# OFA-Sys/ONE-PEACE

Measured on NVIDIA H100. Metric: encoder_samples_per_sec, higher is better.
Workload: dtype bf16

## Files before the change

### one_peace_b200/csrc/gemm_wgmma.cu

```cuda
#include "common.cuh"
#include "gemm.h"

#include <mutex>

namespace opb {

constexpr int kBlockM = 128;
constexpr int kBlockN = 256;
constexpr int kBlockK = 64;
constexpr int kStages = 4;
constexpr int kABytes = kBlockM * kBlockK * 2;
constexpr int kBBytes = kBlockN * kBlockK * 2;
constexpr int kStageBytes = kABytes + kBBytes;
constexpr int kThreads = 384;
constexpr int kBandM = 8;
constexpr int kResidBatch = 16;

struct EpiOperands {
  float2 row[kBlockM];
  float colsum[kBlockN], bias[kBlockN], gamma[kBlockN], colscale[kBlockN];
};
constexpr int kStagerThreads = 96;
constexpr int kSmemBytes = kStages * kStageBytes + 1024 + 2 * sizeof(EpiOperands) + 1024;

struct GemmGeom {
  int M, N, K;
  int kb_inner;
  int num_k_blocks;
  int groups;
  int a_group_c0;
  int b_group_rows;
  int a_mn;
  int b_mn;
  int kb_per_piece;
  int m_pad;
  float* split_ws;
};

OPB_DEVICE void fence_acc(float (&d)[128]) {
#pragma unroll
  for (int i = 0; i < 128; ++i) asm volatile("" : "+f"(d[i])::"memory");
}

template <int TA, int TB>
OPB_DEVICE void wgmma_m64n256k16(float (&d)[128], uint64_t desc_a, uint64_t desc_b, uint32_t scale_d) {
  asm volatile(
      "{\n\t"
      ".reg .pred p;\n\t"
      "setp.ne.b32 p, %130, 0;\n\t"
      "wgmma.mma_async.sync.aligned.m64n256k16.f32.bf16.bf16 "
      "{"
      "%0, %1, %2, %3, %4, %5, %6, %7, %8, %9, %10, %11, %12, %13, %14, %15, "
      "%16, %17, %18, %19, %20, %21, %22, %23, %24, %25, %26, %27, %28, %29, %30, %31, "
      "%32, %33, %34, %35, %36, %37, %38, %39, %40, %41, %42, %43, %44, %45, %46, %47, "
      "%48, %49, %50, %51, %52, %53, %54, %55, %56, %57, %58, %59, %60, %61, %62, %63, "
      "%64, %65, %66, %67, %68, %69, %70, %71, %72, %73, %74, %75, %76, %77, %78, %79, "
      "%80, %81, %82, %83, %84, %85, %86, %87, %88, %89, %90, %91, %92, %93, %94, %95, "
      "%96, %97, %98, %99, %100, %101, %102, %103, %104, %105, %106, %107, %108, %109, %110, %111, "
      "%112, %113, %114, %115, %116, %117, %118, %119, %120, %121, %122, %123, %124, %125, %126, %127"
      "}, %128, %129, p, 1, 1, %131, %132;\n\t"
      "}\n"
      : "+f"(d[0]), "+f"(d[1]), "+f"(d[2]), "+f"(d[3]), "+f"(d[4]), "+f"(d[5]), "+f"(d[6]), "+f"(d[7]),
        "+f"(d[8]), "+f"(d[9]), "+f"(d[10]), "+f"(d[11]), "+f"(d[12]), "+f"(d[13]), "+f"(d[14]), "+f"(d[15]),
        "+f"(d[16]), "+f"(d[17]), "+f"(d[18]), "+f"(d[19]), "+f"(d[20]), "+f"(d[21]), "+f"(d[22]), "+f"(d[23]),
        "+f"(d[24]), "+f"(d[25]), "+f"(d[26]), "+f"(d[27]), "+f"(d[28]), "+f"(d[29]), "+f"(d[30]), "+f"(d[31]),
        "+f"(d[32]), "+f"(d[33]), "+f"(d[34]), "+f"(d[35]), "+f"(d[36]), "+f"(d[37]), "+f"(d[38]), "+f"(d[39]),
        "+f"(d[40]), "+f"(d[41]), "+f"(d[42]), "+f"(d[43]), "+f"(d[44]), "+f"(d[45]), "+f"(d[46]), "+f"(d[47]),
        "+f"(d[48]), "+f"(d[49]), "+f"(d[50]), "+f"(d[51]), "+f"(d[52]), "+f"(d[53]), "+f"(d[54]), "+f"(d[55]),
        "+f"(d[56]), "+f"(d[57]), "+f"(d[58]), "+f"(d[59]), "+f"(d[60]), "+f"(d[61]), "+f"(d[62]), "+f"(d[63]),
        "+f"(d[64]), "+f"(d[65]), "+f"(d[66]), "+f"(d[67]), "+f"(d[68]), "+f"(d[69]), "+f"(d[70]), "+f"(d[71]),
        "+f"(d[72]), "+f"(d[73]), "+f"(d[74]), "+f"(d[75]), "+f"(d[76]), "+f"(d[77]), "+f"(d[78]), "+f"(d[79]),
        "+f"(d[80]), "+f"(d[81]), "+f"(d[82]), "+f"(d[83]), "+f"(d[84]), "+f"(d[85]), "+f"(d[86]), "+f"(d[87]),
        "+f"(d[88]), "+f"(d[89]), "+f"(d[90]), "+f"(d[91]), "+f"(d[92]), "+f"(d[93]), "+f"(d[94]), "+f"(d[95]),
        "+f"(d[96]), "+f"(d[97]), "+f"(d[98]), "+f"(d[99]), "+f"(d[100]), "+f"(d[101]), "+f"(d[102]), "+f"(d[103]),
        "+f"(d[104]), "+f"(d[105]), "+f"(d[106]), "+f"(d[107]), "+f"(d[108]), "+f"(d[109]), "+f"(d[110]), "+f"(d[111]),
        "+f"(d[112]), "+f"(d[113]), "+f"(d[114]), "+f"(d[115]), "+f"(d[116]), "+f"(d[117]), "+f"(d[118]), "+f"(d[119]),
        "+f"(d[120]), "+f"(d[121]), "+f"(d[122]), "+f"(d[123]), "+f"(d[124]), "+f"(d[125]), "+f"(d[126]), "+f"(d[127])
      : "l"(desc_a), "l"(desc_b), "r"(scale_d), "n"(TA), "n"(TB));
}

template <bool kFusedVar = false>
OPB_DEVICE void load_ln_stats(const GemmEpilogue& ep, int row, int M, float& mu, float& rs) {
  mu = 0.f; rs = 1.f;
  const int rc = row < M ? row : M - 1;
  if (ep.ln_partial != nullptr) {
    float s1 = 0.f, s2 = 0.f;
#pragma unroll 8
    for (int p = 0; p < ep.ln_parts; ++p) {
      const float2 v = *reinterpret_cast<const float2*>(ep.ln_partial + (static_cast<long>(p) * M + rc) * 2);
      s1 += v.x; s2 += v.y;
    }
    mu = s1 / ep.ln_dim;
    const float ex2 = s2 / ep.ln_dim;
    const float var = kFusedVar ? fmaf(-mu, mu, ex2) : __fsub_rn(ex2, __fmul_rn(mu, mu));
    rs = rsqrtf(fmaxf(var, 0.f) + ep.ln_eps);
  } else if (ep.ln_mu != nullptr) {
    mu = ep.ln_mu[rc];
    rs = ep.ln_rstd[rc];
  }
}

OPB_DEVICE float2 ldf2(const float* p) { return *reinterpret_cast<const float2*>(p); }
OPB_DEVICE float quad_sum(float v) {
  v += __shfl_xor_sync(0xffffffffu, v, 1);
  return v + __shfl_xor_sync(0xffffffffu, v, 2);
}

template <int TA, int TB>
OPB_DEVICE void mainloop(float (&d)[128], uint8_t* smem, uint64_t* full, uint64_t* empty, int num_k_blocks, int cw,
                         uint32_t it0) {
  constexpr uint32_t step_a = TA ? 2048 : 32, step_b = TB ? 2048 : 32;
  const bool signal = (threadIdx.x & 31) == 0;
  for (int kb = 0; kb < num_k_blocks; ++kb) {
    const uint32_t it = it0 + kb;
    const uint32_t s = it % kStages;
    mbar_wait_quiet(&full[s], (it / kStages) & 1);
    const uint32_t sa = smem_u32(smem + s * kStageBytes) + cw * 8192;
    const uint32_t sb = smem_u32(smem + s * kStageBytes + kABytes);
    fence_acc(d);
    wgmma_fence();
#pragma unroll
    for (int k = 0; k < kBlockK / 16; ++k)
      wgmma_m64n256k16<TA, TB>(d, wgmma_desc_sw128(sa + k * step_a, 8192), wgmma_desc_sw128(sb + k * step_b, 8192),
                               (kb > 0 || k > 0) ? 1u : 0u);
    wgmma_commit();
    fence_acc(d);
    if (kb > 0) {
      wgmma_wait<1>();
      fence_acc(d);
      __syncwarp();
      if (signal) mbar_arrive(&empty[(it - 1) % kStages]);
    }
  }
  wgmma_wait<0>();
  fence_acc(d);
  __syncwarp();
  if (signal) mbar_arrive(&empty[(it0 + num_k_blocks - 1) % kStages]);
}

constexpr bool epi_staged(int epi) { return epi != EPI_LSE_PARTIAL && epi != EPI_SOFTMAX_GRAD; }

template <int EPI>
OPB_DEVICE void stage_epi_operands(EpiOperands* st, const GemmEpilogue& ep, const GemmGeom& geo, int m_blk, int n_blk, int grp,
                                   int t) {
  if (ep.ln_partial != nullptr || ep.ln_mu != nullptr) {
    for (int r = t; r < kBlockM; r += kStagerThreads) {
      float mu, rs;
      load_ln_stats<EPI == EPI_GEGLU_BF16 || EPI == EPI_RESID_F32>(ep, m_blk * kBlockM + r, geo.M, mu, rs);
      st->row[r] = make_float2(mu, rs);
    }
  }
  for (int c = t; c < kBlockN; c += kStagerThreads) {
    const int tc = n_blk * kBlockN + c;
    const bool ok = tc < geo.N;
    const int col = grp * geo.N + tc;
    st->colsum[c] = ok && ep.ln_colsum != nullptr ? ep.ln_colsum[col] : 0.f;
    st->bias[c] = ok && ep.bias != nullptr ? ep.bias[col] : 0.f;
    st->gamma[c] = ok && ep.gamma != nullptr ? ep.gamma[col] : 0.f;
    st->colscale[c] = ok && ep.colscale != nullptr ? ep.colscale[col] : 0.f;
  }
}

template <int EPI>
OPB_DEVICE void epilogue(const float (&d)[128], const GemmEpilogue& ep, const GemmGeom& geo, const EpiOperands* st, int m_blk,
                         int n_blk, int grp, int cw) {
  const int M = geo.M, N = geo.N;
  const int t = threadIdx.x & 127;
  const int lane = t & 31;
  const int quad = lane & 3;
  const int rloc = cw * 64 + (t >> 5) * 16 + (lane >> 2);
  const int rbase = m_blk * kBlockM + rloc;
  const int col0 = n_blk * kBlockN;
  const int gcol0 = grp * N;
#pragma unroll
  for (int h = 0; h < 2; ++h) {
    const int row = rbase + 8 * h;
    bool row_ok = row < M;
    if (ep.out_group > 0 && ep.out_group_valid > 0 && (row % ep.out_group) >= ep.out_group_valid) row_ok = false;
    long out_row = row;
    if (ep.out_group > 0) out_row = static_cast<long>(row / ep.out_group) * ep.out_group_stride + (row % ep.out_group) + ep.out_row_offset;
    long res_row = out_row;
    if (ep.resid_period > 0) res_row = (row % ep.resid_period) + ep.resid_row_offset;

    if constexpr (EPI == EPI_LSE_PARTIAL) {
      const float scale = *ep.scale_ptr;
      const int tgt = row + ep.target_offset;
      const int nv = ep.n_valid > 0 ? ep.n_valid : N;
      float m = -INFINITY;
#pragma unroll
      for (int j = 0; j < 32; ++j) {
        const int col = col0 + 8 * j + 2 * quad;
        if (col < nv) m = fmaxf(m, scale * d[4 * j + 2 * h]);
        if (col + 1 < nv) m = fmaxf(m, scale * d[4 * j + 2 * h + 1]);
      }
      float ssum = 0.f, zsum = 0.f, best = -INFINITY, ztgt = 0.f;
      int best_idx = 0, has_tgt = 0;
#pragma unroll
      for (int j = 0; j < 32; ++j) {
#pragma unroll
        for (int e = 0; e < 2; ++e) {
          const int col = col0 + 8 * j + 2 * quad + e;
          if (col < nv) {
            const float z = scale * d[4 * j + 2 * h + e];
            ssum += __expf(z - m);
            zsum += z;
            if (z > best) { best = z; best_idx = col; }
            if (col == tgt) { ztgt = z; has_tgt = 1; }
          }
        }
      }
#pragma unroll
      for (int o = 1; o <= 2; o <<= 1) {
        const float m2 = __shfl_xor_sync(0xffffffffu, m, o), s2 = __shfl_xor_sync(0xffffffffu, ssum, o);
        const float zs2 = __shfl_xor_sync(0xffffffffu, zsum, o), b2 = __shfl_xor_sync(0xffffffffu, best, o);
        const int i2 = __shfl_xor_sync(0xffffffffu, best_idx, o), h2 = __shfl_xor_sync(0xffffffffu, has_tgt, o);
        const float zt2 = __shfl_xor_sync(0xffffffffu, ztgt, o);
        const float mn = fmaxf(m, m2);
        ssum = (m > -INFINITY ? ssum * __expf(m - mn) : 0.f) + (m2 > -INFINITY ? s2 * __expf(m2 - mn) : 0.f);
        m = mn;
        zsum += zs2;
        if (b2 > best || (b2 == best && i2 < best_idx)) { best = b2; best_idx = i2; }
        if (h2) { ztgt = zt2; has_tgt = 1; }
      }
      if (row_ok && quad == 0) {
        float* w = ep.ws + (static_cast<long>(n_blk) * M + row) * 8;
        *reinterpret_cast<float4*>(w) = make_float4(m, ssum, zsum, best);
        *reinterpret_cast<float4*>(w + 4) = make_float4(__int_as_float(best_idx), ztgt, has_tgt ? 1.f : 0.f, 0.f);
      }
    } else if constexpr (EPI == EPI_SOFTMAX_GRAD) {
      const float scale = *ep.scale_ptr;
      const float gscale = scale * ep.coef;
      const int tgt = row + ep.target_offset;
      const float lse = row_ok ? ep.row_lse[row] : 0.f;
      const float hit = 1.f - ep.eps - ep.eps_i;
      const int nv = ep.n_valid > 0 ? ep.n_valid : N;
      float gz = 0.f;
#pragma unroll
      for (int j = 0; j < 32; ++j) {
        const int col = col0 + 8 * j + 2 * quad;
        if (!row_ok || col >= N) continue;
        float gq[2];
#pragma unroll
        for (int e = 0; e < 2; ++e) {
          const float z = scale * d[4 * j + 2 * h + e];
          float g = __expf(z - lse) - ep.eps_i;
          if (col + e == tgt) g -= hit;
          if (col + e >= nv) g = 0.f;
          gz += g * z;
          gq[e] = g * gscale;
        }
        *reinterpret_cast<uint32_t*>(reinterpret_cast<__nv_bfloat16*>(ep.out) + out_row * ep.ldo + col) = pack_bf16x2(gq[0], gq[1]);
      }
      gz = quad_sum(gz);
      if (row_ok && quad == 0) ep.ws[static_cast<long>(n_blk) * M + row] = gz;
    } else {
      const float2 mr = (ep.ln_partial != nullptr || ep.ln_mu != nullptr) ? st->row[rloc + 8 * h] : make_float2(0.f, 1.f);
      const float mu = mr.x, rs = mr.y;
      const bool has_ln = ep.ln_colsum != nullptr;
      float st_sum = 0.f, st_sq = 0.f;
      if constexpr (EPI == EPI_GEGLU_BF16) {
        __nv_bfloat16* out = reinterpret_cast<__nv_bfloat16*>(ep.out) + out_row * ep.ldo + n_blk * (kBlockN / 2);
#pragma unroll
        for (int j = 0; j < 16; ++j) {
          const int tc = 8 * j + 2 * quad;
          float g0 = d[4 * j + 2 * h], g1 = d[4 * j + 2 * h + 1];
          float l0 = d[4 * (j + 16) + 2 * h], l1 = d[4 * (j + 16) + 2 * h + 1];
          if (has_ln) {
            const float2 cg = ldf2(st->colsum + tc), cl = ldf2(st->colsum + tc + kBlockN / 2);
            g0 = rs * (g0 - mu * cg.x); g1 = rs * (g1 - mu * cg.y);
            l0 = rs * (l0 - mu * cl.x); l1 = rs * (l1 - mu * cl.y);
          }
          if (ep.bias != nullptr) {
            const float2 bg = ldf2(st->bias + tc), bl = ldf2(st->bias + tc + kBlockN / 2);
            g0 += bg.x; g1 += bg.y; l0 += bl.x; l1 += bl.y;
          }
          const float u0 = gelu_erf(g0) * l0, u1 = gelu_erf(g1) * l1;
          st_sum += u0 + u1;
          st_sq += u0 * u0 + u1 * u1;
          if (row_ok) *reinterpret_cast<uint32_t*>(out + tc) = pack_bf16x2(u0, u1);
        }
        st_sum = quad_sum(st_sum);
        st_sq = quad_sum(st_sq);
        if (row_ok && quad == 0 && ep.stats_out != nullptr) {
          *reinterpret_cast<float2*>(ep.stats_out + (static_cast<long>(n_blk * 2) * M + row) * 2) = make_float2(st_sum, st_sq);
          *reinterpret_cast<float2*>(ep.stats_out + (static_cast<long>(n_blk * 2 + 1) * M + row) * 2) = make_float2(0.f, 0.f);
        }
      } else {
#pragma unroll
        for (int jb = 0; jb < 32; jb += kResidBatch) {
          float2 res[kResidBatch];
          if constexpr (EPI == EPI_RESID_F32) {
            if (ep.resid != nullptr && row_ok) {
              const float* rp = ep.resid + res_row * ep.ldr + gcol0;
#pragma unroll
              for (int jj = 0; jj < kResidBatch; ++jj) {
                const int tc = col0 + 8 * (jb + jj) + 2 * quad;
                if (tc < N) res[jj] = ldf2(rp + tc);
              }
            }
          }
#pragma unroll
          for (int jj = 0; jj < kResidBatch; ++jj) {
            const int j = jb + jj;
            const int lc = 8 * j + 2 * quad;
            const int tc = col0 + lc;
            if (tc >= N) continue;
            const int col = gcol0 + tc;
            float x0 = d[4 * j + 2 * h], x1 = d[4 * j + 2 * h + 1];
            if (has_ln) {
              const float2 c = ldf2(st->colsum + lc);
              x0 = rs * (x0 - mu * c.x); x1 = rs * (x1 - mu * c.y);
            }
            if (ep.bias != nullptr) {
              const float2 b = ldf2(st->bias + lc);
              x0 += b.x; x1 += b.y;
            }
            if constexpr (EPI == EPI_STORE_BF16 || EPI == EPI_GELU_BF16) {
              if (ep.colscale != nullptr) {
                const float2 s = ldf2(st->colscale + lc);
                x0 *= s.x; x1 *= s.y;
              }
              if constexpr (EPI == EPI_GELU_BF16) { x0 = gelu_erf(x0); x1 = gelu_erf(x1); }
              if (row_ok) *reinterpret_cast<uint32_t*>(reinterpret_cast<__nv_bfloat16*>(ep.out) + out_row * ep.ldo + col) = pack_bf16x2(x0, x1);
            } else {
              if constexpr (EPI == EPI_RESID_F32) {
                if (ep.gamma != nullptr) {
                  const float2 g = ldf2(st->gamma + lc);
                  x0 *= g.x; x1 *= g.y;
                }
                if (ep.resid != nullptr && row_ok) {
                  x0 += res[jj].x; x1 += res[jj].y;
                }
                st_sum += x0 + x1;
                st_sq += x0 * x0 + x1 * x1;
                if (row_ok && ep.out_bf16 != nullptr)
                  *reinterpret_cast<uint32_t*>(reinterpret_cast<__nv_bfloat16*>(ep.out_bf16) + out_row * ep.ldo_bf16 + col) = pack_bf16x2(x0, x1);
              }
              if (row_ok) *reinterpret_cast<float2*>(reinterpret_cast<float*>(ep.out) + out_row * ep.ldo + col) = make_float2(x0, x1);
            }
          }
        }
        if constexpr (EPI == EPI_RESID_F32) {
          st_sum = quad_sum(st_sum);
          st_sq = quad_sum(st_sq);
          if (row_ok && quad == 0 && ep.stats_out != nullptr)
            *reinterpret_cast<float2*>(ep.stats_out + (static_cast<long>(n_blk) * M + row) * 2) = make_float2(st_sum, st_sq);
        }
      }
    }
  }
}

struct TileCoord {
  int piece, grp, m_blk, n_blk;
};
OPB_DEVICE TileCoord tile_coord(int unit, int num_m_tiles, int num_n_tiles, int groups) {
  const int per_group = num_m_tiles * num_n_tiles;
  TileCoord c;
  c.piece = unit / (per_group * groups);
  const int tile = unit - c.piece * per_group * groups;
  c.grp = tile / per_group;
  const int tin = tile - c.grp * per_group;
  const int band = tin / (kBandM * num_n_tiles);
  const int m0 = band * kBandM;
  const int band_rows = min(kBandM, num_m_tiles - m0);
  const int r = tin - m0 * num_n_tiles;
  c.m_blk = m0 + r % band_rows;
  c.n_blk = r / band_rows;
  return c;
}

template <int EPI>
__global__ void __launch_bounds__(kThreads, 1)
gemm_bf16_kernel(const __grid_constant__ CUtensorMap tm_a, const __grid_constant__ CUtensorMap tm_b, const GemmEpilogue ep,
                 const GemmGeom geo) {
  extern __shared__ __align__(1024) uint8_t smem_raw[];
  uint8_t* smem = smem_raw;
  if ((smem_u32(smem) & 1023u) != 0) __trap();
  uint64_t* full = reinterpret_cast<uint64_t*>(smem + kStages * kStageBytes);
  uint64_t* empty = full + kStages;
  uint64_t* epi_full = empty + kStages;
  uint64_t* epi_empty = epi_full + 2;
  EpiOperands* epi_ops = reinterpret_cast<EpiOperands*>(smem + kStages * kStageBytes + 1024);

  const int wg = threadIdx.x >> 7;
  const int num_m_tiles = (geo.M + kBlockM - 1) / kBlockM;
  const int num_n_tiles = (geo.N + kBlockN - 1) / kBlockN;
  const int pieces = geo.kb_per_piece > 0 ? (geo.num_k_blocks + geo.kb_per_piece - 1) / geo.kb_per_piece : 1;
  const int units = num_m_tiles * num_n_tiles * geo.groups * pieces;
  const bool staged = epi_staged(EPI) && geo.kb_per_piece == 0;

  if (threadIdx.x == 0) {
    tma_prefetch_desc(&tm_a);
    tma_prefetch_desc(&tm_b);
    for (int i = 0; i < kStages; ++i) {
      mbar_init(&full[i], 1);
      mbar_init(&empty[i], 8);
    }
    for (int i = 0; i < 2; ++i) {
      mbar_init(&epi_full[i], kStagerThreads);
      mbar_init(&epi_empty[i], 8);
    }
    fence_barrier_init();
  }
  __syncthreads();

  if (wg == 0) {
    asm volatile("setmaxnreg.dec.sync.aligned.u32 40;");
    if (threadIdx.x == 0) {
      uint32_t it = 0;
      for (int unit = blockIdx.x; unit < units; unit += gridDim.x) {
        const TileCoord tc = tile_coord(unit, num_m_tiles, num_n_tiles, geo.groups);
        const int kb0 = geo.kb_per_piece > 0 ? tc.piece * geo.kb_per_piece : 0;
        const int kb1 = geo.kb_per_piece > 0 ? min(geo.num_k_blocks, kb0 + geo.kb_per_piece) : geo.num_k_blocks;
        const int a_row = tc.m_blk * kBlockM;
        const int b_row = tc.grp * geo.b_group_rows + tc.n_blk * kBlockN;
        const int a_c0 = tc.grp * geo.a_group_c0;
        int kin = kb0 % geo.kb_inner, tap = kb0 / geo.kb_inner;
        for (int kb = kb0; kb < kb1; ++kb, ++it) {
          const uint32_t s = it % kStages;
          mbar_wait_quiet(&empty[s], ((it / kStages) & 1) ^ 1);
          uint8_t* sa = smem + s * kStageBytes;
          uint8_t* sb = sa + kABytes;
          mbar_arrive_expect_tx(&full[s], kStageBytes);
          if (geo.a_mn) {
#pragma unroll
            for (int i = 0; i < kBlockM / 64; ++i) tma_load_2d(&tm_a, &full[s], sa + i * 8192, a_row + 64 * i, kb * kBlockK);
          } else {
            tma_load_3d(&tm_a, &full[s], sa, a_c0 + kin * kBlockK, tap, a_row);
          }
          if (geo.b_mn) {
#pragma unroll
            for (int i = 0; i < kBlockN / 64; ++i) tma_load_2d(&tm_b, &full[s], sb + i * 8192, b_row + 64 * i, kb * kBlockK);
          } else {
            tma_load_2d(&tm_b, &full[s], sb, kb * kBlockK, b_row);
          }
          if (++kin == geo.kb_inner) { kin = 0; ++tap; }
        }
      }
    } else if (threadIdx.x >= 32 && staged) {
      uint32_t j = 0;
      for (int unit = blockIdx.x; unit < units; unit += gridDim.x, ++j) {
        const TileCoord tc = tile_coord(unit, num_m_tiles, num_n_tiles, geo.groups);
        mbar_wait_quiet(&epi_empty[j & 1], ((j >> 1) & 1) ^ 1);
        stage_epi_operands<EPI>(&epi_ops[j & 1], ep, geo, tc.m_blk, tc.n_blk, tc.grp, threadIdx.x - 32);
        mbar_arrive(&epi_full[j & 1]);
      }
    }
  } else {
    asm volatile("setmaxnreg.inc.sync.aligned.u32 232;");
    const int cw = wg - 1;
    float d[128];
#pragma unroll
    for (int i = 0; i < 128; ++i) d[i] = 0.f;
    uint32_t it = 0, j = 0;
    for (int unit = blockIdx.x; unit < units; unit += gridDim.x, ++j) {
      const TileCoord tc = tile_coord(unit, num_m_tiles, num_n_tiles, geo.groups);
      const int kb0 = geo.kb_per_piece > 0 ? tc.piece * geo.kb_per_piece : 0;
      const int kb1 = geo.kb_per_piece > 0 ? min(geo.num_k_blocks, kb0 + geo.kb_per_piece) : geo.num_k_blocks;
      if (geo.a_mn) {
        if (geo.b_mn) mainloop<1, 1>(d, smem, full, empty, kb1 - kb0, cw, it);
        else mainloop<1, 0>(d, smem, full, empty, kb1 - kb0, cw, it);
      } else {
        if (geo.b_mn) mainloop<0, 1>(d, smem, full, empty, kb1 - kb0, cw, it);
        else mainloop<0, 0>(d, smem, full, empty, kb1 - kb0, cw, it);
      }
      it += kb1 - kb0;
      if (geo.kb_per_piece > 0) {
        const int t = threadIdx.x & 127, lane = t & 31;
        const int r0 = tc.m_blk * kBlockM + cw * 64 + (t >> 5) * 16 + (lane >> 2);
        float* w = geo.split_ws + static_cast<long>(tc.piece) * geo.m_pad * geo.N;
#pragma unroll
        for (int h = 0; h < 2; ++h) {
#pragma unroll
          for (int c = 0; c < 32; ++c) {
            const int col = tc.n_blk * kBlockN + 8 * c + 2 * (lane & 3);
            if (col < geo.N)
              *reinterpret_cast<float2*>(w + static_cast<long>(r0 + 8 * h) * geo.N + col) = make_float2(d[4 * c + 2 * h], d[4 * c + 2 * h + 1]);
          }
        }
      } else if (staged) {
        mbar_wait_quiet(&epi_full[j & 1], (j >> 1) & 1);
        epilogue<EPI>(d, ep, geo, &epi_ops[j & 1], tc.m_blk, tc.n_blk, tc.grp, cw);
        __syncwarp();
        if ((threadIdx.x & 31) == 0) mbar_arrive(&epi_empty[j & 1]);
      } else {
        epilogue<EPI>(d, ep, geo, nullptr, tc.m_blk, tc.n_blk, tc.grp, cw);
      }
    }
  }
}

__global__ void __launch_bounds__(256)
gemm_split_epilogue_kernel(const GemmEpilogue ep, const GemmGeom geo, int pieces, int epi) {
  __shared__ float red[2][8];
  const int M = geo.M, N = geo.N;
  const int row = blockIdx.x;
  float mu, rs;
  if (ep.ln_partial != nullptr) {
    float s1 = 0.f, s2 = 0.f;
    for (int p = threadIdx.x; p < ep.ln_parts; p += blockDim.x) {
      const float2 v = *reinterpret_cast<const float2*>(ep.ln_partial + (static_cast<long>(p) * M + row) * 2);
      s1 += v.x; s2 += v.y;
    }
    s1 = warp_sum(s1); s2 = warp_sum(s2);
    if ((threadIdx.x & 31) == 0) { red[0][threadIdx.x >> 5] = s1; red[1][threadIdx.x >> 5] = s2; }
    __syncthreads();
    s1 = s2 = 0.f;
    for (int i = 0; i < 8; ++i) { s1 += red[0][i]; s2 += red[1][i]; }
    mu = s1 / ep.ln_dim;
    rs = rsqrtf(fmaxf(s2 / ep.ln_dim - mu * mu, 0.f) + ep.ln_eps);
  } else {
    load_ln_stats(ep, row, M, mu, rs);
  }
  const int t = blockIdx.y;
  const int col = t * kBlockN + threadIdx.x;
  const long slab = static_cast<long>(geo.m_pad) * N;
  float x = 0.f;
  if (col < N) {
    const float* w = geo.split_ws + static_cast<long>(row) * N + col;
    for (int p = 0; p < pieces; ++p) x += w[p * slab];
    if (ep.ln_colsum) x = rs * (x - mu * ep.ln_colsum[col]);
    if (ep.bias) x += ep.bias[col];
    if (epi == EPI_STORE_BF16) {
      if (ep.colscale) x *= ep.colscale[col];
      reinterpret_cast<__nv_bfloat16*>(ep.out)[static_cast<long>(row) * ep.ldo + col] = __float2bfloat16(x);
    } else {
      if (ep.gamma) x *= ep.gamma[col];
      if (ep.resid) x += ep.resid[static_cast<long>(row) * ep.ldr + col];
      reinterpret_cast<float*>(ep.out)[static_cast<long>(row) * ep.ldo + col] = x;
      if (ep.out_bf16) reinterpret_cast<__nv_bfloat16*>(ep.out_bf16)[static_cast<long>(row) * ep.ldo_bf16 + col] = __float2bfloat16(x);
    }
  }
  if (ep.stats_out != nullptr) {
    const float s1 = warp_sum(x), s2 = warp_sum(x * x);
    __syncthreads();
    if ((threadIdx.x & 31) == 0) { red[0][threadIdx.x >> 5] = s1; red[1][threadIdx.x >> 5] = s2; }
    __syncthreads();
    if (threadIdx.x == 0) {
      float a = 0.f, b = 0.f;
      for (int i = 0; i < 8; ++i) { a += red[0][i]; b += red[1][i]; }
      *reinterpret_cast<float2*>(ep.stats_out + (static_cast<long>(t) * M + row) * 2) = make_float2(a, b);
    }
  }
}

typedef CUresult (*PFN_encodeTiled)(CUtensorMap*, CUtensorMapDataType, cuuint32_t, void*, const cuuint64_t*,
                                    const cuuint64_t*, const cuuint32_t*, const cuuint32_t*, CUtensorMapInterleave,
                                    CUtensorMapSwizzle, CUtensorMapL2promotion, CUtensorMapFloatOOBfill);

static PFN_encodeTiled get_encode_fn() {
  static PFN_encodeTiled fn = nullptr;
  static std::once_flag once;
  std::call_once(once, [] {
    void* p = nullptr;
    cudaDriverEntryPointQueryResult qres;
    if (cudaGetDriverEntryPoint("cuTensorMapEncodeTiled", &p, cudaEnableDefault, &qres) == cudaSuccess &&
        qres == cudaDriverEntryPointSuccess) {
      fn = reinterpret_cast<PFN_encodeTiled>(p);
    }
  });
  return fn;
}

int make_tmap_bf16_2d(CUtensorMap* out, const void* ptr, uint64_t rows, uint64_t cols, uint64_t ld,
                      uint32_t box_rows) {
  PFN_encodeTiled enc = get_encode_fn();
  if (enc == nullptr) return OPB_ERR_CUDA;
  if ((reinterpret_cast<uintptr_t>(ptr) & 15) != 0 || (ld * 2) % 16 != 0) return OPB_ERR_INVALID;
  cuuint64_t gdim[2] = {cols, rows};
  cuuint64_t gstride[1] = {ld * 2};
  cuuint32_t box[2] = {static_cast<cuuint32_t>(kBlockK), box_rows};
  cuuint32_t estr[2] = {1, 1};
  CUresult r = enc(out, CU_TENSOR_MAP_DATA_TYPE_BFLOAT16, 2, const_cast<void*>(ptr), gdim, gstride, box, estr,
                   CU_TENSOR_MAP_INTERLEAVE_NONE, CU_TENSOR_MAP_SWIZZLE_128B, CU_TENSOR_MAP_L2_PROMOTION_L2_256B,
                   CU_TENSOR_MAP_FLOAT_OOB_FILL_NONE);
  return r == CUDA_SUCCESS ? OPB_OK : OPB_ERR_CUDA;
}

int make_tmap_bf16_3d(CUtensorMap* out, const void* ptr, uint64_t k_inner, uint64_t taps, uint64_t tap_stride,
                      uint64_t rows, uint64_t row_stride, uint32_t box_rows) {
  PFN_encodeTiled enc = get_encode_fn();
  if (enc == nullptr) return OPB_ERR_CUDA;
  if ((reinterpret_cast<uintptr_t>(ptr) & 15) != 0 || (tap_stride * 2) % 16 != 0 || (row_stride * 2) % 16 != 0)
    return OPB_ERR_INVALID;
  cuuint64_t gdim[3] = {k_inner, taps, rows};
  cuuint64_t gstride[2] = {tap_stride * 2, row_stride * 2};
  cuuint32_t box[3] = {static_cast<cuuint32_t>(kBlockK), 1, box_rows};
  cuuint32_t estr[3] = {1, 1, 1};
  CUresult r = enc(out, CU_TENSOR_MAP_DATA_TYPE_BFLOAT16, 3, const_cast<void*>(ptr), gdim, gstride, box, estr,
                   CU_TENSOR_MAP_INTERLEAVE_NONE, CU_TENSOR_MAP_SWIZZLE_128B, CU_TENSOR_MAP_L2_PROMOTION_L2_256B,
                   CU_TENSOR_MAP_FLOAT_OOB_FILL_NONE);
  return r == CUDA_SUCCESS ? OPB_OK : OPB_ERR_CUDA;
}

int make_tmap_bf16_batched(CUtensorMap* out, const void* ptr, uint64_t cols, uint64_t rows, uint64_t ld, uint64_t batches,
                           uint64_t batch_stride, uint32_t box_rows) {
  PFN_encodeTiled enc = get_encode_fn();
  if (enc == nullptr) return OPB_ERR_CUDA;
  if ((reinterpret_cast<uintptr_t>(ptr) & 15) != 0 || (ld * 2) % 16 != 0 || (batch_stride * 2) % 16 != 0)
    return OPB_ERR_INVALID;
  cuuint64_t gdim[3] = {cols, rows, batches};
  cuuint64_t gstride[2] = {ld * 2, batch_stride * 2};
  cuuint32_t box[3] = {static_cast<cuuint32_t>(kBlockK), box_rows, 1};
  cuuint32_t estr[3] = {1, 1, 1};
  CUresult r = enc(out, CU_TENSOR_MAP_DATA_TYPE_BFLOAT16, 3, const_cast<void*>(ptr), gdim, gstride, box, estr,
                   CU_TENSOR_MAP_INTERLEAVE_NONE, CU_TENSOR_MAP_SWIZZLE_128B, CU_TENSOR_MAP_L2_PROMOTION_L2_256B,
                   CU_TENSOR_MAP_FLOAT_OOB_FILL_NONE);
  return r == CUDA_SUCCESS ? OPB_OK : OPB_ERR_CUDA;
}

template <int EPI>
static int launch_gemm(const CUtensorMap& ta, const CUtensorMap& tb, const GemmEpilogue& ep, const GemmGeom& geo,
                       cudaStream_t stream) {
  auto kern = gemm_bf16_kernel<EPI>;
  static int resident = 0;
  if (resident == 0) {
    if (cudaFuncSetAttribute(kern, cudaFuncAttributeMaxDynamicSharedMemorySize, kSmemBytes) != cudaSuccess)
      return OPB_ERR_CUDA;
    int per_sm = 0;
    if (cudaOccupancyMaxActiveBlocksPerMultiprocessor(&per_sm, kern, kThreads, kSmemBytes) != cudaSuccess || per_sm < 1)
      return OPB_ERR_CUDA;
    resident = per_sm * sm_count();
  }
  const int pieces = geo.kb_per_piece > 0 ? (geo.num_k_blocks + geo.kb_per_piece - 1) / geo.kb_per_piece : 1;
  const long units = static_cast<long>((geo.M + kBlockM - 1) / kBlockM) * ((geo.N + kBlockN - 1) / kBlockN) * geo.groups * pieces;
  const unsigned grid = static_cast<unsigned>(units < resident ? units : resident);
  kern<<<grid, kThreads, kSmemBytes, stream>>>(ta, tb, ep, geo);
  return cudaGetLastError() == cudaSuccess ? OPB_OK : OPB_ERR_CUDA;
}

static int dispatch_gemm(int epi, const CUtensorMap& ta, const CUtensorMap& tb, const GemmEpilogue& ep, const GemmGeom& geo,
                         cudaStream_t stream) {
  switch (epi) {
    case EPI_STORE_BF16: return launch_gemm<EPI_STORE_BF16>(ta, tb, ep, geo, stream);
    case EPI_GELU_BF16: return launch_gemm<EPI_GELU_BF16>(ta, tb, ep, geo, stream);
    case EPI_GEGLU_BF16: return launch_gemm<EPI_GEGLU_BF16>(ta, tb, ep, geo, stream);
    case EPI_RESID_F32: return launch_gemm<EPI_RESID_F32>(ta, tb, ep, geo, stream);
    case EPI_STORE_F32: return launch_gemm<EPI_STORE_F32>(ta, tb, ep, geo, stream);
    case EPI_LSE_PARTIAL: return launch_gemm<EPI_LSE_PARTIAL>(ta, tb, ep, geo, stream);
    case EPI_SOFTMAX_GRAD: return launch_gemm<EPI_SOFTMAX_GRAD>(ta, tb, ep, geo, stream);
    default: return OPB_ERR_INVALID;
  }
}

struct ByteSpan {
  const char* begin;
  const char* end;
};
static ByteSpan row_span(const void* p, long lo, long hi, long ld, long cols, int esz) {
  const char* c = static_cast<const char*>(p);
  return {c + lo * ld * esz, c + (hi * ld + cols) * esz};
}
static bool spans_meet(const ByteSpan& a, const ByteSpan& b) { return a.begin < b.end && b.begin < a.end; }

static bool resid_aliasing_ok(const GemmEpilogue& ep, int M, long cols) {
  if (ep.resid == nullptr) return true;
  auto out_row = [&](long m) {
    return ep.out_group > 0 ? (m / ep.out_group) * ep.out_group_stride + m % ep.out_group + ep.out_row_offset : m;
  };
  const long g = ep.out_group > 0 ? ep.out_group : M, last = M - 1, q = last / g;
  const long corners[5] = {0, (g < M ? g : M) - 1, q * g, last, q > 0 ? q * g - 1 : 0};
  long lo = out_row(0), hi = lo;
  for (long m : corners) {
    lo = out_row(m) < lo ? out_row(m) : lo;
    hi = out_row(m) > hi ? out_row(m) : hi;
  }
  long rlo = lo, rhi = hi;
  if (ep.resid_period > 0) {
    rlo = ep.resid_row_offset;
    rhi = rlo + (ep.resid_period < M ? ep.resid_period : M) - 1;
  }
  const ByteSpan res = row_span(ep.resid, rlo, rhi, ep.ldr, cols, 4);
  if (ep.out_bf16 != nullptr && spans_meet(res, row_span(ep.out_bf16, lo, hi, ep.ldo_bf16, cols, 2))) return false;
  if (!spans_meet(res, row_span(ep.out, lo, hi, ep.ldo, cols, 4))) return true;
  return ep.resid == ep.out && ep.ldr == ep.ldo && ep.resid_period == 0;
}

static GemmGeom plain_geom(int M, int N, int K) {
  GemmGeom geo;
  geo.M = M; geo.N = N; geo.K = K;
  geo.num_k_blocks = (K + kBlockK - 1) / kBlockK;
  geo.kb_inner = geo.num_k_blocks;
  geo.groups = 1;
  geo.a_group_c0 = 0;
  geo.b_group_rows = 0;
  geo.a_mn = geo.b_mn = 0;
  geo.kb_per_piece = 0;
  geo.m_pad = 0;
  geo.split_ws = nullptr;
  return geo;
}

int gemm_bf16(const void* A, int lda, const void* B, int ldb, int M, int N, int K, int epi, const GemmEpilogue& ep,
              int cta_group, cudaStream_t stream) {
  if (M <= 0 || N <= 0 || K <= 0) return OPB_ERR_INVALID;
  if (K % 8 != 0 || N % 8 != 0 || lda % 8 != 0 || ldb % 8 != 0) return OPB_ERR_INVALID;
  if (epi == EPI_GEGLU_BF16 && N % kBlockN != 0) return OPB_ERR_INVALID;
  if (cta_group < 0 || cta_group > 2) return OPB_ERR_INVALID;
  if (epi == EPI_RESID_F32 && !resid_aliasing_ok(ep, M, N)) return OPB_ERR_INVALID;
  GemmGeom geo = plain_geom(M, N, K);
  const int m_tiles = (M + kBlockM - 1) / kBlockM, n_tiles = (N + kBlockN - 1) / kBlockN;
  const bool split_ok = (epi == EPI_RESID_F32 || (epi == EPI_STORE_BF16 && ep.stats_out == nullptr)) && ep.workspace != nullptr &&
                        ep.out_group == 0 && ep.resid_period == 0 && M <= 2 * kBlockM && geo.num_k_blocks >= 8;
  int pieces = 1;
  if (split_ok) {
    const long slab_bytes = static_cast<long>(m_tiles) * kBlockM * N * 4;
    pieces = sm_count() / (m_tiles * n_tiles);
    if (pieces > geo.num_k_blocks / 2) pieces = geo.num_k_blocks / 2;
    if (pieces > ep.workspace_bytes / slab_bytes) pieces = static_cast<int>(ep.workspace_bytes / slab_bytes);
    if (pieces >= 2) {
      geo.kb_per_piece = (geo.num_k_blocks + pieces - 1) / pieces;
      pieces = (geo.num_k_blocks + geo.kb_per_piece - 1) / geo.kb_per_piece;
      geo.m_pad = m_tiles * kBlockM;
      geo.split_ws = reinterpret_cast<float*>(ep.workspace);
    }
  }
  CUtensorMap ta, tb;
  int rc = make_tmap_bf16_3d(&ta, A, K, 1, lda, M, lda, kBlockM);
  if (rc != OPB_OK) return rc;
  rc = make_tmap_bf16_2d(&tb, B, N, K, ldb, kBlockN);
  if (rc != OPB_OK) return rc;
  rc = dispatch_gemm(epi, ta, tb, ep, geo, stream);
  if (rc != OPB_OK || geo.kb_per_piece == 0) return rc;
  gemm_split_epilogue_kernel<<<dim3(M, n_tiles), 256, 0, stream>>>(ep, geo, pieces, epi);
  return cudaGetLastError() == cudaSuccess ? OPB_OK : OPB_ERR_CUDA;
}

int gemm_bf16_t(const void* A, int lda, int a_mn, const void* B, int ldb, int b_mn, int M, int N, int K, int epi,
                const GemmEpilogue& ep, int cta_group, cudaStream_t stream) {
  if (M <= 0 || N <= 0 || K <= 0 || lda % 8 != 0 || ldb % 8 != 0 || N % 8 != 0) return OPB_ERR_INVALID;
  if (epi != EPI_STORE_BF16 && epi != EPI_STORE_F32) return OPB_ERR_INVALID;
  if ((!a_mn && K % 8 != 0) || (!b_mn && K % 8 != 0) || (a_mn && M % 8 != 0)) return OPB_ERR_INVALID;
  if (cta_group < 0 || cta_group > 2) return OPB_ERR_INVALID;
  GemmGeom geo = plain_geom(M, N, K);
  geo.a_mn = a_mn ? 1 : 0;
  geo.b_mn = b_mn ? 1 : 0;
  CUtensorMap ta, tb;
  int rc = a_mn ? make_tmap_bf16_2d(&ta, A, K, M, lda, 64) : make_tmap_bf16_3d(&ta, A, K, 1, lda, M, lda, kBlockM);
  if (rc != OPB_OK) return rc;
  rc = b_mn ? make_tmap_bf16_2d(&tb, B, K, N, ldb, 64) : make_tmap_bf16_2d(&tb, B, N, K, ldb, kBlockN);
  if (rc != OPB_OK) return rc;
  return dispatch_gemm(epi, ta, tb, ep, geo, stream);
}

int gemm_bf16_grouped_window(const void* X, const void* W, int rows, int groups, int c_pad, int taps, int n_per_group,
                             int epi, const GemmEpilogue& ep, cudaStream_t stream) {
  if (rows <= 0 || groups <= 0 || taps <= 0 || n_per_group <= 0) return OPB_ERR_INVALID;
  if (c_pad % kBlockK != 0 || n_per_group % 8 != 0 || n_per_group > kBlockN) return OPB_ERR_INVALID;
  if (epi == EPI_GEGLU_BF16 || epi == EPI_LSE_PARTIAL || epi == EPI_SOFTMAX_GRAD) return OPB_ERR_INVALID;
  if (epi == EPI_RESID_F32 && !resid_aliasing_ok(ep, rows, static_cast<long>(groups) * n_per_group)) return OPB_ERR_INVALID;
  GemmGeom geo = plain_geom(rows, n_per_group, taps * c_pad);
  geo.kb_inner = c_pad / kBlockK;
  geo.num_k_blocks = taps * geo.kb_inner;
  geo.groups = groups;
  geo.a_group_c0 = c_pad;
  geo.b_group_rows = n_per_group;
  const long row_stride = static_cast<long>(groups) * c_pad;
  CUtensorMap ta, tb;
  int rc = make_tmap_bf16_3d(&ta, X, row_stride, taps, row_stride, rows, row_stride, kBlockM);
  if (rc != OPB_OK) return rc;
  rc = make_tmap_bf16_2d(&tb, W, static_cast<uint64_t>(groups) * n_per_group, geo.K, geo.K, kBlockN);
  if (rc != OPB_OK) return rc;
  return dispatch_gemm(epi, ta, tb, ep, geo, stream);
}

}
```

Before: 762.9.

## Stage bf16 GEMM epilogue outputs through shared memory and TMA bulk stores

Adds a TMA-store variant of the persistent wgmma GEMM for bf16 epilogues (store, GELU, GEGLU). Each consumer warpgroup packs its output with stmatrix into a swizzled shared-memory staging buffer and issues 2D TMA stores, in place of scattered 4-byte global writes. To make room in shared memory the stage ring drops from 4 to 3, which reduces how far loads can run ahead of the math. A warpgroup barrier and a bulk-read wait guard reuse of the staging buffer.

After: 790.7, median of 6. +3.6%, better.

```diff
diff --git a/one_peace_b200/csrc/gemm_wgmma.cu b/one_peace_b200/csrc/gemm_wgmma.cu
--- a/one_peace_b200/csrc/gemm_wgmma.cu
+++ b/one_peace_b200/csrc/gemm_wgmma.cu
@@ -9,6 +9,7 @@
 constexpr int kBlockN = 256;
 constexpr int kBlockK = 64;
 constexpr int kStages = 4;
+constexpr int kStagesTmaOut = 3;
 constexpr int kABytes = kBlockM * kBlockK * 2;
 constexpr int kBBytes = kBlockN * kBlockK * 2;
 constexpr int kStageBytes = kABytes + kBBytes;
@@ -21,7 +22,14 @@
   float colsum[kBlockN], bias[kBlockN], gamma[kBlockN], colscale[kBlockN];
 };
 constexpr int kStagerThreads = 96;
-constexpr int kSmemBytes = kStages * kStageBytes + 1024 + 2 * sizeof(EpiOperands) + 1024;
+constexpr int kOutBoxBytes = 64 * 128;
+constexpr int kOutStageBytes = 4 * kOutBoxBytes;
+constexpr int smem_bytes(int stages, bool tma_out) {
+  return stages * kStageBytes + (tma_out ? 2 * kOutStageBytes : 0) + 1024 + 2 * sizeof(EpiOperands) + 1024;
+}
+constexpr int kSmemBytes = smem_bytes(kStages, false);
+constexpr int kSmemBytesTmaOut = smem_bytes(kStagesTmaOut, true);
+static_assert(kSmemBytesTmaOut <= 227 * 1024, "output staging does not fit next to the stage ring");
 
 struct GemmGeom {
   int M, N, K;
@@ -106,15 +114,15 @@
   return v + __shfl_xor_sync(0xffffffffu, v, 2);
 }
 
-template <int TA, int TB>
+template <int TA, int TB, int S>
 OPB_DEVICE void mainloop(float (&d)[128], uint8_t* smem, uint64_t* full, uint64_t* empty, int num_k_blocks, int cw,
                          uint32_t it0) {
   constexpr uint32_t step_a = TA ? 2048 : 32, step_b = TB ? 2048 : 32;
   const bool signal = (threadIdx.x & 31) == 0;
   for (int kb = 0; kb < num_k_blocks; ++kb) {
     const uint32_t it = it0 + kb;
-    const uint32_t s = it % kStages;
-    mbar_wait_quiet(&full[s], (it / kStages) & 1);
+    const uint32_t s = it % S;
+    mbar_wait_quiet(&full[s], (it / S) & 1);
     const uint32_t sa = smem_u32(smem + s * kStageBytes) + cw * 8192;
     const uint32_t sb = smem_u32(smem + s * kStageBytes + kABytes);
     fence_acc(d);
@@ -129,13 +137,49 @@
       wgmma_wait<1>();
       fence_acc(d);
       __syncwarp();
-      if (signal) mbar_arrive(&empty[(it - 1) % kStages]);
+      if (signal) mbar_arrive(&empty[(it - 1) % S]);
     }
   }
   wgmma_wait<0>();
   fence_acc(d);
   __syncwarp();
-  if (signal) mbar_arrive(&empty[(it0 + num_k_blocks - 1) % kStages]);
+  if (signal) mbar_arrive(&empty[(it0 + num_k_blocks - 1) % S]);
+}
+
+template <int kGroups>
+OPB_DEVICE void stage_out_row(uint32_t stage, int h, const uint32_t (&v)[kGroups]) {
+  const int lane = threadIdx.x & 31;
+  const int row = ((threadIdx.x & 127) >> 5) * 16 + 8 * h + (lane & 7);
+#pragma unroll
+  for (int q = 0; q < kGroups / 4; ++q) {
+    const int cg = 4 * q + (lane >> 3);
+    const uint32_t addr = stage + (cg >> 3) * kOutBoxBytes + sw128_off(row, cg & 7);
+    asm volatile("stmatrix.sync.aligned.m8n8.x4.shared.b16 [%0], {%1, %2, %3, %4};" ::"r"(addr), "r"(v[4 * q]),
+                 "r"(v[4 * q + 1]), "r"(v[4 * q + 2]), "r"(v[4 * q + 3]));
+  }
+}
+
+OPB_DEVICE void warpgroup_bar_sync(int cw) {
+  if (cw == 0) asm volatile("bar.sync 1, 128;" ::: "memory");
+  else asm volatile("bar.sync 2, 128;" ::: "memory");
+}
+
+OPB_DEVICE void acquire_out_stage(int cw) {
+  if ((threadIdx.x & 127) == 0) bulk_wait_read<0>();
+  warpgroup_bar_sync(cw);
+}
+
+OPB_DEVICE void store_out_tile(const CUtensorMap& tm_out, uint8_t* stage, int row0, int col0, int rows, int cols, int boxes,
+                               int cw) {
+  fence_proxy_async();
+  warpgroup_bar_sync(cw);
+  if ((threadIdx.x & 127) == 0) {
+    if (row0 < rows) {
+      for (int b = 0; b < boxes; ++b)
+        if (col0 + 64 * b < cols) tma_store_2d(&tm_out, stage + b * kOutBoxBytes, col0 + 64 * b, row0);
+    }
+    bulk_commit();
+  }
 }
 
 constexpr bool epi_staged(int epi) { return epi != EPI_LSE_PARTIAL && epi != EPI_SOFTMAX_GRAD; }
@@ -161,9 +205,9 @@
   }
 }
 
-template <int EPI>
-OPB_DEVICE void epilogue(const float (&d)[128], const GemmEpilogue& ep, const GemmGeom& geo, const EpiOperands* st, int m_blk,
-                         int n_blk, int grp, int cw) {
+template <int EPI, bool kTmaOut>
+OPB_DEVICE void epilogue(const float (&d)[128], const GemmEpilogue& ep, const GemmGeom& geo, const EpiOperands* st,
+                         uint32_t out_stage, int m_blk, int n_blk, int grp, int cw) {
   const int M = geo.M, N = geo.N;
   const int t = threadIdx.x & 127;
   const int lane = t & 31;
@@ -260,6 +304,7 @@
       float st_sum = 0.f, st_sq = 0.f;
       if constexpr (EPI == EPI_GEGLU_BF16) {
         __nv_bfloat16* out = reinterpret_cast<__nv_bfloat16*>(ep.out) + out_row * ep.ldo + n_blk * (kBlockN / 2);
+        uint32_t packed[16];
 #pragma unroll
         for (int j = 0; j < 16; ++j) {
           const int tc = 8 * j + 2 * quad;
@@ -277,8 +322,10 @@
           const float u0 = gelu_erf(g0) * l0, u1 = gelu_erf(g1) * l1;
           st_sum += u0 + u1;
           st_sq += u0 * u0 + u1 * u1;
-          if (row_ok) *reinterpret_cast<uint32_t*>(out + tc) = pack_bf16x2(u0, u1);
+          if constexpr (kTmaOut) packed[j] = pack_bf16x2(u0, u1);
+          else if (row_ok) *reinterpret_cast<uint32_t*>(out + tc) = pack_bf16x2(u0, u1);
         }
+        if constexpr (kTmaOut) stage_out_row(out_stage, h, packed);
         st_sum = quad_sum(st_sum);
         st_sq = quad_sum(st_sq);
         if (row_ok && quad == 0 && ep.stats_out != nullptr) {
@@ -286,6 +333,7 @@
           *reinterpret_cast<float2*>(ep.stats_out + (static_cast<long>(n_blk * 2 + 1) * M + row) * 2) = make_float2(0.f, 0.f);
         }
       } else {
+        uint32_t packed[32];
 #pragma unroll
         for (int jb = 0; jb < 32; jb += kResidBatch) {
           float2 res[kResidBatch];
@@ -304,7 +352,7 @@
             const int j = jb + jj;
             const int lc = 8 * j + 2 * quad;
             const int tc = col0 + lc;
-            if (tc >= N) continue;
+            if (!kTmaOut && tc >= N) continue;
             const int col = gcol0 + tc;
             float x0 = d[4 * j + 2 * h], x1 = d[4 * j + 2 * h + 1];
             if (has_ln) {
@@ -321,7 +369,11 @@
                 x0 *= s.x; x1 *= s.y;
               }
               if constexpr (EPI == EPI_GELU_BF16) { x0 = gelu_erf(x0); x1 = gelu_erf(x1); }
-              if (row_ok) *reinterpret_cast<uint32_t*>(reinterpret_cast<__nv_bfloat16*>(ep.out) + out_row * ep.ldo + col) = pack_bf16x2(x0, x1);
+              if constexpr (kTmaOut) {
+                packed[j] = pack_bf16x2(x0, x1);
+              } else {
+                if (row_ok) *reinterpret_cast<uint32_t*>(reinterpret_cast<__nv_bfloat16*>(ep.out) + out_row * ep.ldo + col) = pack_bf16x2(x0, x1);
+              }
             } else {
               if constexpr (EPI == EPI_RESID_F32) {
                 if (ep.gamma != nullptr) {
@@ -340,6 +392,7 @@
             }
           }
         }
+        if constexpr (kTmaOut) stage_out_row(out_stage, h, packed);
         if constexpr (EPI == EPI_RESID_F32) {
           st_sum = quad_sum(st_sum);
           st_sq = quad_sum(st_sq);
@@ -370,30 +423,32 @@
   return c;
 }
 
-template <int EPI>
-__global__ void __launch_bounds__(kThreads, 1)
-gemm_bf16_kernel(const __grid_constant__ CUtensorMap tm_a, const __grid_constant__ CUtensorMap tm_b, const GemmEpilogue ep,
-                 const GemmGeom geo) {
+template <int EPI, int S, bool kTmaOut>
+OPB_DEVICE void gemm_body(const CUtensorMap& tm_a, const CUtensorMap& tm_b, const CUtensorMap* tm_out, const GemmEpilogue& ep,
+                          const GemmGeom& geo) {
   extern __shared__ __align__(1024) uint8_t smem_raw[];
   uint8_t* smem = smem_raw;
   if ((smem_u32(smem) & 1023u) != 0) __trap();
-  uint64_t* full = reinterpret_cast<uint64_t*>(smem + kStages * kStageBytes);
-  uint64_t* empty = full + kStages;
-  uint64_t* epi_full = empty + kStages;
+  uint8_t* out_stage = smem + S * kStageBytes;
+  uint8_t* bars = out_stage + (kTmaOut ? 2 * kOutStageBytes : 0);
+  uint64_t* full = reinterpret_cast<uint64_t*>(bars);
+  uint64_t* empty = full + S;
+  uint64_t* epi_full = empty + S;
   uint64_t* epi_empty = epi_full + 2;
-  EpiOperands* epi_ops = reinterpret_cast<EpiOperands*>(smem + kStages * kStageBytes + 1024);
+  EpiOperands* epi_ops = reinterpret_cast<EpiOperands*>(bars + 1024);
 
   const int wg = threadIdx.x >> 7;
   const int num_m_tiles = (geo.M + kBlockM - 1) / kBlockM;
   const int num_n_tiles = (geo.N + kBlockN - 1) / kBlockN;
   const int pieces = geo.kb_per_piece > 0 ? (geo.num_k_blocks + geo.kb_per_piece - 1) / geo.kb_per_piece : 1;
   const int units = num_m_tiles * num_n_tiles * geo.groups * pieces;
-  const bool staged = epi_staged(EPI) && geo.kb_per_piece == 0;
+  const bool staged = epi_staged(EPI) && (kTmaOut || geo.kb_per_piece == 0);
 
   if (threadIdx.x == 0) {
     tma_prefetch_desc(&tm_a);
     tma_prefetch_desc(&tm_b);
-    for (int i = 0; i < kStages; ++i) {
+    if constexpr (kTmaOut) tma_prefetch_desc(tm_out);
+    for (int i = 0; i < S; ++i) {
       mbar_init(&full[i], 1);
       mbar_init(&empty[i], 8);
     }
@@ -418,8 +473,8 @@
         const int a_c0 = tc.grp * geo.a_group_c0;
         int kin = kb0 % geo.kb_inner, tap = kb0 / geo.kb_inner;
         for (int kb = kb0; kb < kb1; ++kb, ++it) {
-          const uint32_t s = it % kStages;
-          mbar_wait_quiet(&empty[s], ((it / kStages) & 1) ^ 1);
+          const uint32_t s = it % S;
+          mbar_wait_quiet(&empty[s], ((it / S) & 1) ^ 1);
           uint8_t* sa = smem + s * kStageBytes;
           uint8_t* sb = sa + kABytes;
           mbar_arrive_expect_tx(&full[s], kStageBytes);
@@ -450,6 +505,7 @@
   } else {
     asm volatile("setmaxnreg.inc.sync.aligned.u32 232;");
     const int cw = wg - 1;
+    uint8_t* my_stage = out_stage + cw * kOutStageBytes;
     float d[128];
 #pragma unroll
     for (int i = 0; i < 128; ++i) d[i] = 0.f;
@@ -459,14 +515,14 @@
       const int kb0 = geo.kb_per_piece > 0 ? tc.piece * geo.kb_per_piece : 0;
       const int kb1 = geo.kb_per_piece > 0 ? min(geo.num_k_blocks, kb0 + geo.kb_per_piece) : geo.num_k_blocks;
       if (geo.a_mn) {
-        if (geo.b_mn) mainloop<1, 1>(d, smem, full, empty, kb1 - kb0, cw, it);
-        else mainloop<1, 0>(d, smem, full, empty, kb1 - kb0, cw, it);
+        if (geo.b_mn) mainloop<1, 1, S>(d, smem, full, empty, kb1 - kb0, cw, it);
+        else mainloop<1, 0, S>(d, smem, full, empty, kb1 - kb0, cw, it);
       } else {
-        if (geo.b_mn) mainloop<0, 1>(d, smem, full, empty, kb1 - kb0, cw, it);
-        else mainloop<0, 0>(d, smem, full, empty, kb1 - kb0, cw, it);
+        if (geo.b_mn) mainloop<0, 1, S>(d, smem, full, empty, kb1 - kb0, cw, it);
+        else mainloop<0, 0, S>(d, smem, full, empty, kb1 - kb0, cw, it);
       }
       it += kb1 - kb0;
-      if (geo.kb_per_piece > 0) {
+      if (!kTmaOut && geo.kb_per_piece > 0) {
         const int t = threadIdx.x & 127, lane = t & 31;
         const int r0 = tc.m_blk * kBlockM + cw * 64 + (t >> 5) * 16 + (lane >> 2);
         float* w = geo.split_ws + static_cast<long>(tc.piece) * geo.m_pad * geo.N;
@@ -481,14 +537,38 @@
         }
       } else if (staged) {
         mbar_wait_quiet(&epi_full[j & 1], (j >> 1) & 1);
-        epilogue<EPI>(d, ep, geo, &epi_ops[j & 1], tc.m_blk, tc.n_blk, tc.grp, cw);
+        if constexpr (kTmaOut) acquire_out_stage(cw);
+        epilogue<EPI, kTmaOut>(d, ep, geo, &epi_ops[j & 1], smem_u32(my_stage), tc.m_blk, tc.n_blk, tc.grp, cw);
         __syncwarp();
         if ((threadIdx.x & 31) == 0) mbar_arrive(&epi_empty[j & 1]);
+        if constexpr (kTmaOut) {
+          constexpr int cols_per_tile = EPI == EPI_GEGLU_BF16 ? kBlockN / 2 : kBlockN;
+          store_out_tile(*tm_out, my_stage, tc.m_blk * kBlockM + cw * 64, tc.n_blk * cols_per_tile, geo.M,
+                         EPI == EPI_GEGLU_BF16 ? geo.N / 2 : geo.N, cols_per_tile / 64, cw);
+        }
       } else {
-        epilogue<EPI>(d, ep, geo, nullptr, tc.m_blk, tc.n_blk, tc.grp, cw);
-      }
-    }
-  }
+        epilogue<EPI, false>(d, ep, geo, nullptr, 0, tc.m_blk, tc.n_blk, tc.grp, cw);
+      }
+    }
+    if constexpr (kTmaOut) {
+      if ((threadIdx.x & 127) == 0) bulk_wait_all<0>();
+    }
+  }
+}
+
+template <int EPI>
+__global__ void __launch_bounds__(kThreads, 1)
+gemm_bf16_kernel(const __grid_constant__ CUtensorMap tm_a, const __grid_constant__ CUtensorMap tm_b, const GemmEpilogue ep,
+                 const GemmGeom geo) {
+  gemm_body<EPI, kStages, false>(tm_a, tm_b, nullptr, ep, geo);
+}
+
+template <int EPI>
+__global__ void __launch_bounds__(kThreads, 1)
+gemm_bf16_tma_out_kernel(const __grid_constant__ CUtensorMap tm_a, const __grid_constant__ CUtensorMap tm_b,
+                         const __grid_constant__ CUtensorMap tm_out, const GemmEpilogue ep, const GemmGeom geo) {
+  static_assert(EPI == EPI_STORE_BF16 || EPI == EPI_GELU_BF16 || EPI == EPI_GEGLU_BF16, "bf16 epilogues only");
+  gemm_body<EPI, kStagesTmaOut, true>(tm_a, tm_b, &tm_out, ep, geo);
 }
 
 __global__ void __launch_bounds__(256)
@@ -610,38 +690,55 @@
   return r == CUDA_SUCCESS ? OPB_OK : OPB_ERR_CUDA;
 }
 
-template <int EPI>
-static int launch_gemm(const CUtensorMap& ta, const CUtensorMap& tb, const GemmEpilogue& ep, const GemmGeom& geo,
-                       cudaStream_t stream) {
-  auto kern = gemm_bf16_kernel<EPI>;
+template <int EPI, bool kTmaOut>
+static int launch_gemm(const CUtensorMap& ta, const CUtensorMap& tb, const CUtensorMap* to, const GemmEpilogue& ep,
+                       const GemmGeom& geo, cudaStream_t stream) {
+  constexpr int smem = kTmaOut ? kSmemBytesTmaOut : kSmemBytes;
+  const void* kern;
+  if constexpr (kTmaOut) kern = reinterpret_cast<const void*>(gemm_bf16_tma_out_kernel<EPI>);
+  else kern = reinterpret_cast<const void*>(gemm_bf16_kernel<EPI>);
   static int resident = 0;
   if (resident == 0) {
-    if (cudaFuncSetAttribute(kern, cudaFuncAttributeMaxDynamicSharedMemorySize, kSmemBytes) != cudaSuccess)
+    if (cudaFuncSetAttribute(kern, cudaFuncAttributeMaxDynamicSharedMemorySize, smem) != cudaSuccess)
       return OPB_ERR_CUDA;
     int per_sm = 0;
-    if (cudaOccupancyMaxActiveBlocksPerMultiprocessor(&per_sm, kern, kThreads, kSmemBytes) != cudaSuccess || per_sm < 1)
+    if (cudaOccupancyMaxActiveBlocksPerMultiprocessor(&per_sm, kern, kThreads, smem) != cudaSuccess || per_sm < 1)
       return OPB_ERR_CUDA;
     resident = per_sm * sm_count();
   }
   const int pieces = geo.kb_per_piece > 0 ? (geo.num_k_blocks + geo.kb_per_piece - 1) / geo.kb_per_piece : 1;
   const long units = static_cast<long>((geo.M + kBlockM - 1) / kBlockM) * ((geo.N + kBlockN - 1) / kBlockN) * geo.groups * pieces;
   const unsigned grid = static_cast<unsigned>(units < resident ? units : resident);
-  kern<<<grid, kThreads, kSmemBytes, stream>>>(ta, tb, ep, geo);
+  if constexpr (kTmaOut) gemm_bf16_tma_out_kernel<EPI><<<grid, kThreads, smem, stream>>>(ta, tb, *to, ep, geo);
+  else gemm_bf16_kernel<EPI><<<grid, kThreads, smem, stream>>>(ta, tb, ep, geo);
   return cudaGetLastError() == cudaSuccess ? OPB_OK : OPB_ERR_CUDA;
 }
 
-static int dispatch_gemm(int epi, const CUtensorMap& ta, const CUtensorMap& tb, const GemmEpilogue& ep, const GemmGeom& geo,
-                         cudaStream_t stream) {
+static int dispatch_gemm(int epi, const CUtensorMap& ta, const CUtensorMap& tb, const CUtensorMap* to, const GemmEpilogue& ep,
+                         const GemmGeom& geo, cudaStream_t stream) {
+  if (to != nullptr) {
+    switch (epi) {
+      case EPI_STORE_BF16: return launch_gemm<EPI_STORE_BF16, true>(ta, tb, to, ep, geo, stream);
+      case EPI_GELU_BF16: return launch_gemm<EPI_GELU_BF16, true>(ta, tb, to, ep, geo, stream);
+      case EPI_GEGLU_BF16: return launch_gemm<EPI_GEGLU_BF16, true>(ta, tb, to, ep, geo, stream);
+      default: return OPB_ERR_INVALID;
+    }
+  }
   switch (epi) {
-    case EPI_STORE_BF16: return launch_gemm<EPI_STORE_BF16>(ta, tb, ep, geo, stream);
-    case EPI_GELU_BF16: return launch_gemm<EPI_GELU_BF16>(ta, tb, ep, geo, stream);
-    case EPI_GEGLU_BF16: return launch_gemm<EPI_GEGLU_BF16>(ta, tb, ep, geo, stream);
-    case EPI_RESID_F32: return launch_gemm<EPI_RESID_F32>(ta, tb, ep, geo, stream);
-    case EPI_STORE_F32: return launch_gemm<EPI_STORE_F32>(ta, tb, ep, geo, stream);
-    case EPI_LSE_PARTIAL: return launch_gemm<EPI_LSE_PARTIAL>(ta, tb, ep, geo, stream);
-    case EPI_SOFTMAX_GRAD: return launch_gemm<EPI_SOFTMAX_GRAD>(ta, tb, ep, geo, stream);
+    case EPI_STORE_BF16: return launch_gemm<EPI_STORE_BF16, false>(ta, tb, nullptr, ep, geo, stream);
+    case EPI_GELU_BF16: return launch_gemm<EPI_GELU_BF16, false>(ta, tb, nullptr, ep, geo, stream);
+    case EPI_GEGLU_BF16: return launch_gemm<EPI_GEGLU_BF16, false>(ta, tb, nullptr, ep, geo, stream);
+    case EPI_RESID_F32: return launch_gemm<EPI_RESID_F32, false>(ta, tb, nullptr, ep, geo, stream);
+    case EPI_STORE_F32: return launch_gemm<EPI_STORE_F32, false>(ta, tb, nullptr, ep, geo, stream);
+    case EPI_LSE_PARTIAL: return launch_gemm<EPI_LSE_PARTIAL, false>(ta, tb, nullptr, ep, geo, stream);
+    case EPI_SOFTMAX_GRAD: return launch_gemm<EPI_SOFTMAX_GRAD, false>(ta, tb, nullptr, ep, geo, stream);
     default: return OPB_ERR_INVALID;
   }
+}
+
+static bool tma_out_applies(int epi, const GemmEpilogue& ep, const GemmGeom& geo, long out_cols) {
+  return (epi == EPI_STORE_BF16 || epi == EPI_GELU_BF16 || epi == EPI_GEGLU_BF16) && geo.kb_per_piece == 0 && geo.groups == 1 &&
+         ep.out_group == 0 && (reinterpret_cast<uintptr_t>(ep.out) & 15) == 0 && (ep.ldo * 2) % 16 == 0 && ep.ldo >= out_cols;
 }
 
 struct ByteSpan {
@@ -721,7 +818,11 @@
   if (rc != OPB_OK) return rc;
   rc = make_tmap_bf16_2d(&tb, B, N, K, ldb, kBlockN);
   if (rc != OPB_OK) return rc;
-  rc = dispatch_gemm(epi, ta, tb, ep, geo, stream);
+  const long out_cols = epi == EPI_GEGLU_BF16 ? N / 2 : N;
+  CUtensorMap to;
+  const bool tma_out = tma_out_applies(epi, ep, geo, out_cols);
+  if (tma_out && (rc = make_tmap_bf16_2d(&to, ep.out, M, out_cols, ep.ldo, 64)) != OPB_OK) return rc;
+  rc = dispatch_gemm(epi, ta, tb, tma_out ? &to : nullptr, ep, geo, stream);
   if (rc != OPB_OK || geo.kb_per_piece == 0) return rc;
   gemm_split_epilogue_kernel<<<dim3(M, n_tiles), 256, 0, stream>>>(ep, geo, pieces, epi);
   return cudaGetLastError() == cudaSuccess ? OPB_OK : OPB_ERR_CUDA;
@@ -741,7 +842,10 @@
   if (rc != OPB_OK) return rc;
   rc = b_mn ? make_tmap_bf16_2d(&tb, B, K, N, ldb, 64) : make_tmap_bf16_2d(&tb, B, N, K, ldb, kBlockN);
   if (rc != OPB_OK) return rc;
-  return dispatch_gemm(epi, ta, tb, ep, geo, stream);
+  CUtensorMap to;
+  const bool tma_out = tma_out_applies(epi, ep, geo, N);
+  if (tma_out && (rc = make_tmap_bf16_2d(&to, ep.out, M, N, ep.ldo, 64)) != OPB_OK) return rc;
+  return dispatch_gemm(epi, ta, tb, tma_out ? &to : nullptr, ep, geo, stream);
 }
 
 int gemm_bf16_grouped_window(const void* X, const void* W, int rows, int groups, int c_pad, int taps, int n_per_group,
@@ -762,7 +866,7 @@
   if (rc != OPB_OK) return rc;
   rc = make_tmap_bf16_2d(&tb, W, static_cast<uint64_t>(groups) * n_per_group, geo.K, geo.K, kBlockN);
   if (rc != OPB_OK) return rc;
-  return dispatch_gemm(epi, ta, tb, ep, geo, stream);
-}
-
-}
+  return dispatch_gemm(epi, ta, tb, nullptr, ep, geo, stream);
+}
+
+}
```
